# gooofy/zerovox

Measured on AMD Instinct MI355X. Metric: audio samples/sec + RTF, 128-phoneme zero-shot synth @22.05kHz, 1/2/4/8 GPU, higher is better.
Workload: dtype f16+bf16

## Files before the change

zerovox_amd/csrc/gemm.hip:

```cpp
#include "mfma_util.h"
#include "zvx_kernels.h"

#include <cstring>
#include <type_traits>

#ifndef ZVX_GEMM_PART
#define ZVX_GEMM_PART 0
#endif
#define ZVX_PART_MAIN (ZVX_GEMM_PART != 2)
#define ZVX_PART_RESFUSE (ZVX_GEMM_PART != 1)
#if ZVX_GEMM_PART == 2
extern thread_local bool zvx_gemm_dry_run;
#else
thread_local hipEvent_t zvx_gemm_ev_start = nullptr, zvx_gemm_ev_stop = nullptr;
thread_local bool zvx_gemm_dry_run = false;
#endif
#define g_dry_run zvx_gemm_dry_run

#define ZVX_LAUNCH(...) do { if (!g_dry_run) ZVX_DISPATCH(__VA_ARGS__); } while (0)

namespace zvx {


#define PITCH 80
// ... 1792 lines not shown
        dim3 grid((a.N / 128) * ((a.M + 255) / 256), a.nbatch);
        size_t lds = ((size_t)(256 + hl + hr) * SLAB_PITCH + 1023) & ~(size_t)1023;
        ZVX_LAUNCH((convslab_kernel<256, 128, 2, 2, true, 2, 0, -1, 160>), grid, dim3(256), lds, stream, a);
        return 7;
    }
    if (a.dtype != DT_F32 && a.N == a.K && !a.K2 && (a.ntaps == 3 || a.ntaps == 5 || a.ntaps == 7 || a.ntaps == 11)) {
        if (a.N == 32 && launch_convreg_c<32, 512, 4, 1, 2>(a, stream)) return 14;
        if (a.N == 64 && launch_convreg_c<64, 256, 2, 2, 2>(a, stream)) return 15;
    }
    if (hl + hr > 64) {
        if (hl + hr <= 160 && a.N % 128 == 0 && a.K % SLAB_KC == 0 && !a.K2 && !a.bflat && !a.flat_win && gemm_epi_mode_of(a) == ZVX_EPI(1, 1, 1)) {
            dim3 grid((a.N / 128) * ((a.M + 255) / 256), a.nbatch);
            const size_t lds = ((size_t)(256 + hl + hr) * SLAB_PITCH + 1023) & ~(size_t)1023;
            if (a.dtype == DT_F16) ZVX_LAUNCH((convslab_kernel<256, 128, 2, 2, true, 2, 0, ZVX_EPI(1, 1, 1), 160, true>), grid, dim3(256), lds, stream, a);
            else ZVX_LAUNCH((convslab_kernel<256, 128, 2, 2, true, 2, 0, ZVX_EPI(1, 1, 1), 160>), grid, dim3(256), lds, stream, a);
            return 7;
        }
        return -4;
    }
    static const int bns[4] = {256, 128, 64, 32};
    static const double eff[4] = {0.95, 1.0, 0.7, 0.4};
    int best = 0; double best_cost = -1;
    for (int i = 0; i < 4; i++) {
        const double cost = (double)((a.N + bns[i] - 1) / bns[i]) * bns[i] / eff[i];
        if (best_cost < 0 || cost < best_cost - 1e-9) { best_cost = cost; best = i; }
    }
    static const int bms[4] = {128, 256, 256, 256};
    const int ncu = num_cus();
    if (g_slab_small >= 2 && a.M <= 64 && a.nbatch * ((a.N + 127) / 128) * 4 <= ncu && a.N >= 64 && hl + hr <= 64) {
        a.bflat = 0;
        dim3 g32((a.N + 31) / 32, a.nbatch);
        const size_t lds32 = (((size_t)(256 + hl + hr) * SLAB_PITCH + 1023) & ~(size_t)1023) + (size_t)8 * 1024;
        launch_slab_variant<256, 32, 4, 1, 2, 8>(a, g32, lds32, stream);
        return 9;
    }
    if (g_slab_small && a.M > 128 && a.N >= 128 && hl + hr <= 64) {
        const long wg256 = (long)((a.N + 127) / 128) * ((a.M + 255) / 256) * a.nbatch;
        if (wg256 * 2 <= ncu) {
            a.bflat = 0;
            const bool r64 = wg256 * 4 <= ncu;
            const int bm = r64 ? 64 : 128;
            dim3 gs(((a.N + 127) / 128) * ((a.M + bm - 1) / bm), a.nbatch);
            size_t lds = ((size_t)(bm + hl + hr) * SLAB_PITCH + 1023) & ~(size_t)1023;
            const size_t stage = (size_t)4 * 32 * (2 * 128 + 16);
            if (lds < stage) lds = stage;
            if (r64) launch_slab_variant<64, 128, 2, 2, 2, 0>(a, gs, lds, stream);
            else launch_slab_variant<128, 128, 2, 2, 2, 0>(a, gs, lds, stream);
            return 22;
        }
    }
    if (a.M <= 128 && a.N >= 128) {
        a.bflat = 0;
        const int wide = ((a.N + 255) / 256) * a.nbatch;
        const bool narrow = wide < 2 * ncu;
        const int bn = narrow ? 128 : 256;
        dim3 grid((a.N + bn - 1) / bn, a.nbatch);
        size_t lds = ((size_t)(128 + hl + hr) * SLAB_PITCH + 1023) & ~(size_t)1023;
        const size_t stage = (size_t)4 * 32 * (2 * 128 + 16);
        if (lds < stage) lds = stage;
        if (narrow && a.M > (g_slab_small ? 32 : 64) && ((a.N + 127) / 128) * a.nbatch < 2 * ncu) {
            dim3 g64(((a.N + 127) / 128) * ((a.M + 63) / 64), a.nbatch);
            launch_slab_variant<64, 128, 2, 2, 2, 0>(a, g64, lds, stream);
            return 22;
        }
        if (narrow) { launch_slab_variant<128, 128, 2, 2, 2, 0>(a, grid, lds, stream); return 22; }
        launch_slab_variant<128, 256, 1, 4, 2, 0>(a, grid, lds, stream);
        return 6;
    }
    if (a.ntaps == 1 && a.N >= 512) {
        const long slots = 2L * ncu;
        auto rounds = [&](int bm_, int bn_) {
            const long ntn_ = (a.N + bn_ - 1) / bn_, utt = ntn_ * ((a.M + bm_ - 1) / bm_) * a.nbatch;
            const long flat = a.bflat ? ntn_ * (((long)a.nbatch * a.bflat + bm_ - 1) / bm_) : utt;
            return ((flat < utt ? flat : utt) + slots - 1) / slots;
        };
        best = rounds(256, 128) <= rounds(128, 256) ? 1 : 0;
    }
    const bool wreg = best <= 1;
    const int ring_slots = wreg ? 0 : (best == 0 ? 4 : 8);
    const int bn = bns[best], bm = bms[best];
    const int ntn = (a.N + bn - 1) / bn;
    if (a.bflat) {
        const long slots = 2L * ncu;
        const long wg_utt = (long)ntn * ((a.M + bm - 1) / bm) * a.nbatch, wg_flat = (long)ntn * (((long)a.nbatch * a.bflat + bm - 1) / bm);
        if ((wg_flat + slots - 1) / slots < (wg_utt + slots - 1) / slots) { a.flat_win = a.bflat; a.flat_rows = a.nbatch * a.bflat; a.M = a.flat_rows; a.nbatch = 1; }
        else a.bflat = 0;
    }
    if (best == 1 && bflat_hint && a.M > 256 && hl + hr <= 64) {
        const long slots = 2L * ncu;
        const long t256 = (long)ntn * ((a.M + 255) / 256) * a.nbatch, t128 = (long)ntn * ((a.M + 127) / 128) * a.nbatch;
        const long eff256 = 2 * ((t256 + slots - 1) / slots), eff128 = (t128 + slots - 1) / slots;
        if (eff128 < eff256) {
            dim3 g128(ntn * ((a.M + 127) / 128), a.nbatch);
            size_t lds128 = ((size_t)(128 + hl + hr) * SLAB_PITCH + 1023) & ~(size_t)1023;
            const size_t stage128 = (size_t)4 * 32 * (2 * 128 + 16);
            if (lds128 < stage128) lds128 = stage128;
            switch (gemm_epi_mode_of(a)) {
                case ZVX_EPI(0, 0, 1): launch_slab_variant<128, 128, 2, 2, 2, 0, ZVX_EPI(0, 0, 1)>(a, g128, lds128, stream); break;
                case ZVX_EPI_DEC(0): launch_slab_variant<128, 128, 2, 2, 2, 0, ZVX_EPI_DEC(0)>(a, g128, lds128, stream); break;
                case ZVX_EPI_DEC(1): launch_slab_variant<128, 128, 2, 2, 2, 0, ZVX_EPI_DEC(1)>(a, g128, lds128, stream); break;
                default: launch_slab_variant<128, 128, 2, 2, 2, 0>(a, g128, lds128, stream);
            }
            return 22;
        }
    }
    const int ntm = (a.M + bm - 1) / bm;
    dim3 grid(ntn * ntm, a.nbatch);
// ... 105 lines not shown
```

zerovox_amd/csrc/pairstream.hip:

```cpp
#include "mfma_util.h"
#include "zvx_kernels.h"

#include <algorithm>
#include <type_traits>

namespace zvx {

#define PS_R 128
#define PS_WD 8
#define PS_XP 256
#define PS_TP 272
#define PS_NDMA 8

#ifndef PS_EXP
#define PS_EXP 0
#endif
#ifndef PS_PD
#define PS_PD 2
#endif
#ifndef PS_PRIO
#define PS_PRIO 1
#endif
#ifndef PS_RES_LDS
#define PS_RES_LDS 1
#endif
#ifndef PS_RPF
#define PS_RPF 2
#endif
#ifndef PS_DMA_TAIL
#define PS_DMA_TAIL 1
#endif
#ifdef PS_PROFILE
#define PS_STAMP(k) do { const unsigned long long t_ = __builtin_readcyclecounter(); tacc[k] += t_ - tlast; tlast = t_; } while (0)
#else
#define PS_STAMP(k) do {} while (0)
#endif

template <int ROLE, int NT, int AM, bool HAS_OUT, bool H16>
__device__ __forceinline__ void ps_role(const PairArgs& a, unsigned char* lds, const int lane, const int ct) {
    constexpr int R = PS_R, H2 = (NT - 1) / 2, NS = 8 * NT, WD = PS_WD;
    constexpr int EPI = (ROLE == 0 && !PS_DMA_TAIL) ? (PS_NDMA + NT - 2) / (NT - 1) : 0;
    static_assert(ROLE == 1 || PS_DMA_TAIL || EPI * (NT - 1) >= PS_NDMA, "DMA slots");
    const int l32 = lane & 31, hi = lane >> 5;
    const int dil = a.dil, H1 = dil * H2, DX = a.DX, DT = a.DT, G0 = a.G0;
    const unsigned tbase = (unsigned)DX * PS_XP;
    const float* const bias_l = (const float*)(lds + tbase + (unsigned)DT * PS_TP) + ROLE * 128;
    const unsigned scratch_l = tbase + (unsigned)DT * PS_TP + 1024;

    const unsigned char* const wq = (const unsigned char*)(ROLE ? a.W2 : a.W1) + (long)ct * NS * 1024;
    const unsigned lane16 = lane * 16;
    u32x4 wreg[WD] = {};
    auto wload = [&](int off, int slot) __attribute__((always_inline)) {
        asm volatile("global_load_dwordx4 %0, %1, %2" : "+v"(wreg[slot]) : "v"(lane16), "s"(wq + off) : "memory");
    };
#pragma unroll
    for (int i = 0; i < WD; i++) wload(i * 1024, i);

    const float slope1 = a.slope1, rinv = a.res_inv_slope, oscale = a.out_scale, oslope = a.slope;
    f32x16 acc[4];
#ifdef PS_PROFILE
    unsigned long long tacc[4] = {0, 0, 0, 0}, tlast = __builtin_readcyclecounter();
#endif

    const int nsegs = a.nseg * a.nbatch;
    for (int seg = blockIdx.x; seg < nsegs; seg += gridDim.x) {
        const int b = seg / a.nseg, sj = seg - b * a.nseg;
        int len = a.len ? a.len[b] : a.M;
        len = __builtin_amdgcn_readfirstlane(len);
        const int seg0 = sj * a.S;
        if (seg0 >= len) continue;
        const int seg_end = min(seg0 + a.S, len);
        const int nb = (seg_end - seg0 + 2 * H2 + R - 1) / R;
        const int c1_0 = seg0 - H2;
        const int xrow0 = c1_0 - H1;
        const unsigned short* const Xb = (const unsigned short*)a.X + (long)b * a.x_bs;

        auto dma_rsrc = [&](int grow, bool real) __attribute__((always_inline)) {
            const unsigned long long pa = (unsigned long long)(Xb + (long)grow * a.ldx);
            int nrec = real ? (len - grow) * a.ldx * 2 : 0; if (nrec < 0) nrec = 0;
            return (i32x4){__builtin_amdgcn_readfirstlane((int)(unsigned)pa), __builtin_amdgcn_readfirstlane((int)((pa >> 32) & 0xffff)),
                           __builtin_amdgcn_readfirstlane(nrec), 0x00020000};
        };
        auto dma_piece = [&](const i32x4& rsrc, int grow, int pos, int pc, bool real) __attribute__((always_inline)) {
            int lv = lane;
            asm volatile("" : "+v"(lv));
            const int rr = lv >> 4, sl = lv & 15;
            int p = pos + 4 * pc; if (p >= DX) p -= DX;
            const int key = (p + rr) & 15;
            int voff = ((4 * pc + rr) * a.ldx + ((sl ^ key) << 3)) * 2;
            if (grow + 4 * pc + rr < 0) voff = -16;
            const unsigned la = __builtin_amdgcn_readfirstlane(real ? (unsigned)p * PS_XP : scratch_l);
            asm volatile("s_mov_b32 m0, %0\n\ts_nop 0\n\tbuffer_load_dwordx4 %1, %2, 0 offen lds" :: "s"(la), "v"(voff), "s"(rsrc) : "memory", "m0");
        };

        int x_rd = 0;
        int x_wr = G0;
        int gx = xrow0 + G0;
        int t_wr = 0;
        int t_rd = DT - 2 * H2;
        int g1 = c1_0;
        int g2 = seg0 - 2 * H2;
        if (ROLE == 0) {
            const i32x4 rs0 = dma_rsrc(xrow0, true);
            for (int pc = ct; pc < G0 / 4; pc += 4) dma_piece(rs0, xrow0, 0, pc, true);
            asm volatile("s_waitcnt vmcnt(0)" ::: "memory");
        }
        asm volatile("s_waitcnt lgkmcnt(0)\n\ts_barrier" ::: "memory");

        auto main_loop = [&](bool dma_real) __attribute__((always_inline)) {
#pragma unroll
            for (int j = 0; j < 4; j++)
#pragma unroll
                for (int e = 0; e < 16; e++) acc[j][e] = 0.f;
            unsigned bs[4], nbs[4], pn = 0, hkn = 0;
            auto bases_common = [&](int u) __attribute__((always_inline)) {
                const int kc = u >= NT ? 1 : 0, tap = u - kc * NT;
                if (ROLE == 0) {
                    pn = x_rd + l32 + tap * dil; pn = min(pn, pn - (unsigned)DX);
                    hkn = (((pn ^ hi) & 15u) << 4) ^ ((unsigned)kc << 7);
                } else {
                    pn = t_rd + l32 + tap; pn = min(pn, pn - (unsigned)DT);
                    hkn = tbase + hi * 16 + kc * 128;
                }
            };
            auto bases_tile = [&](int j, unsigned (&o)[4]) __attribute__((always_inline)) {
                unsigned pj = pn + 32 * j;
                if (ROLE == 0) { pj = min(pj, pj - (unsigned)DX); o[j] = (pj << 8) + hkn; }
                else { pj = min(pj, pj - (unsigned)DT); o[j] = pj * PS_TP + hkn; }
            };
            auto rd1 = [&](uint4& xf, unsigned o, int kk) __attribute__((always_inline)) {
                if (PS_EXP & 2) { asm volatile("" : "=v"(xf)); return; }
                if (PS_EXP & 64) {
                    uint4 dummy;
                    if (ROLE == 0) asm volatile("ds_read_b128 %0, %1" : "=v"(dummy) : "v"(o ^ (unsigned)(kk << 5)));
                    else asm volatile("ds_read_b128 %0, %1" : "=v"(dummy) : "v"(o + kk * 32));
                    asm volatile("" : "=v"(xf));
                    return;
                }
                if (ROLE == 0) asm volatile("ds_read_b128 %0, %1" : "=v"(xf) : "v"(o ^ (unsigned)(kk << 5)));
                else {
                    switch (kk) {
                        case 0: asm volatile("ds_read_b128 %0, %1" : "=v"(xf) : "v"(o)); break;
                        case 1: asm volatile("ds_read_b128 %0, %1 offset:32" : "=v"(xf) : "v"(o)); break;
                        case 2: asm volatile("ds_read_b128 %0, %1 offset:64" : "=v"(xf) : "v"(o)); break;
                        default: asm volatile("ds_read_b128 %0, %1 offset:96" : "=v"(xf) : "v"(o)); break;
                    }
                }
            };
            constexpr int PD = PS_PD;
            static_assert(PD == 1 || PD == 2, "prefetch distance");
            uint4 xs[4][4];
            const i32x4 rsd = PS_DMA_TAIL ? (i32x4){0, 0, 0, 0} : dma_rsrc(gx, dma_real);
            bases_common(0);
#pragma unroll
            for (int j = 0; j < 4; j++) bases_tile(j, bs);
            asm volatile("s_waitcnt lgkmcnt(0)" ::: "memory");
            __builtin_amdgcn_sched_barrier(0);
#pragma unroll
            for (int i = 0; i < PD; i++)
#pragma unroll
                for (int j = 0; j < 4; j++) rd1(xs[i][j], bs[j], i);
            for (int u2 = 0; u2 < NT; u2++) {
                const int next_off = (u2 + 1 == NT ? 0 : (u2 + 1) * (WD * 1024));
#pragma unroll
                for (int h = 0; h < 2; h++) {
                    const int u = 2 * u2 + h;
                    int un = u + 1; if (un == 2 * NT) un = 0;
#pragma unroll
                    for (int kk = 0; kk < 4; kk++) {
                        const int i = h * 4 + kk;
                        asm volatile("s_waitcnt vmcnt(%0) lgkmcnt(%1)" :: "n"(WD - 1 + EPI), "n"(4 * (PD - 1)) : "memory");
                        __builtin_amdgcn_sched_barrier(0);
#pragma unroll
                        for (int j = 0; j < 4; j++) {
                            if (PS_EXP & 32) asm volatile("" : "+v"(acc[j]) : "v"(wreg[i]), "v"(xs[i & 3][j]));
                            else acc[j] = mfma16<H16>(wreg[i], xs[i & 3][j], acc[j]);
                            __builtin_amdgcn_sched_barrier(0);
                            if (kk + PD < 4) rd1(xs[(i + PD) & 3][j], bs[j], kk + PD); else rd1(xs[(i + PD) & 3][j], nbs[j], kk + PD - 4);
                            if (kk == 0 && j == 3) bases_common(un);
                            if (kk == 1) bases_tile(j, nbs);
                            if (j == 3) {
                                if (!(PS_EXP & 1)) wload(next_off + i * 1024, i);
                                if (ROLE == 0 && !PS_DMA_TAIL && !(PS_EXP & 8)) {
#pragma unroll
                                    for (int e = 0; e < EPI; e++)
                                        if (i == (7 * e + 3) / EPI) {
                                            const int pidx = u2 * EPI + e;
                                            dma_piece(rsd, gx, x_wr, ct * PS_NDMA + (pidx < PS_NDMA ? pidx : 0), dma_real && pidx < PS_NDMA);
                                        }
                                }
                            }
                            __builtin_amdgcn_sched_barrier(0);
                        }
                    }
#pragma unroll
                    for (int j = 0; j < 4; j++) bs[j] = nbs[j];
                }
            }
            asm volatile("s_waitcnt lgkmcnt(0)" ::: "memory");
            __builtin_amdgcn_sched_barrier(0);
        };

        auto epilogue_T = [&]() __attribute__((always_inline)) {
            int lv = lane;
            asm volatile("" : "+v"(lv));
            const int l32 = lv & 31, hi = lv >> 5;
            float4 bq[4];
#pragma unroll
            for (int q = 0; q < 4; q++) bq[q] = *(const float4*)(bias_l + ct * 32 + 8 * q + 4 * hi);
#pragma unroll
            for (int j = 0; j < 4; j++) {
                const int g = g1 + 32 * j + l32;
                const bool inside = g >= 0 && g < len;
                unsigned wp = t_wr + 32 * j + l32; wp = min(wp, wp - (unsigned)DT);
                unsigned char* const dst = lds + tbase + wp * PS_TP + (ct * 32 + 4 * hi) * 2;
#pragma unroll
                for (int q = 0; q < 4; q++) {
                    const f32x2 v01 = lrelu2((f32x2){acc[j][4 * q], acc[j][4 * q + 1]} + (f32x2){bq[q].x, bq[q].y}, slope1);
                    const f32x2 v23 = lrelu2((f32x2){acc[j][4 * q + 2], acc[j][4 * q + 3]} + (f32x2){bq[q].z, bq[q].w}, slope1);
                    uint2 pk;
                    pk.x = inside ? pack16<H16>(v01.x, v01.y) : 0u;
                    pk.y = inside ? pack16<H16>(v23.x, v23.y) : 0u;
                    if (!(PS_EXP & 16)) *(uint2*)(dst + q * 16) = pk;
                    else asm volatile("" :: "v"(pk.x), "v"(pk.y), "v"(dst));
                }
            }
        };

        int off[4];
        u32x4 rx[4][2], sx[4][2];
        uint2 rcur[4][4], rnext[4][4];
        auto residual_reads = [&](int blk) __attribute__((always_inline)) {
            int lv = lane;
            asm volatile("" : "+v"(lv));
            unsigned p0 = (unsigned)((long)blk * R % DX) + H1 - H2 + (lv & 31);
            p0 = min(p0, p0 - (unsigned)DX);
#pragma unroll
            for (int j = 0; j < 4; j++) {
                unsigned pj = p0 + 32 * j; pj = min(pj, pj - (unsigned)DX);
                const unsigned char* row = lds + pj * PS_XP + (lv >> 5) * 8;
#pragma unroll
                for (int q = 0; q < 4; q++) rnext[j][q] = *(const uint2*)(row + (((ct * 4 + q) ^ (pj & 15u)) << 4));
            }
        };
        auto res_rsrc = [&](const void* base, long bs_) __attribute__((always_inline)) {
            return __builtin_amdgcn_make_buffer_rsrc((void*)((unsigned short*)base + (long)b * bs_), 0, len * a.ldx * 2, 0x00020000);
        };
        auto epilogue_loads = [&](int gb) __attribute__((always_inline)) {
            int lv = lane;
            asm volatile("" : "+v"(lv));
            const int cA = ct * 32 + 8 * (lv >> 5);
            const __amdgpu_buffer_rsrc_t rsX = res_rsrc(a.X, a.x_bs), rsA = res_rsrc(a.accum, a.a_bs);
#pragma unroll
            for (int j = 0; j < 4; j++) {
                const int g = gb + 32 * j + (lv & 31);
                off[j] = (g >= seg0 && g < seg_end && !(PS_EXP & 4)) ? (g * a.ldx + cA) * 2 : (int)0x80000000;
                if (!PS_RES_LDS) {
                    rx[j][0] = __builtin_amdgcn_raw_buffer_load_b128(rsX, off[j], 0, 0);
                    rx[j][1] = __builtin_amdgcn_raw_buffer_load_b128(rsX, off[j] + 32, 0, 0);
                }
            }
            if (AM & 1) {
#pragma unroll
                for (int j = 0; j < 4; j++) {
                    sx[j][0] = __builtin_amdgcn_raw_buffer_load_b128(rsA, off[j], 0, 0);
                    sx[j][1] = __builtin_amdgcn_raw_buffer_load_b128(rsA, off[j] + 32, 0, 0);
                }
            }
        };
        auto epilogue_out = [&]() __attribute__((always_inline)) {
            int lv = lane;
            asm volatile("" : "+v"(lv));
            float4 bq[4];
#pragma unroll
            for (int q = 0; q < 4; q++) bq[q] = *(const float4*)(bias_l + ct * 32 + 8 * q + 4 * (lv >> 5));
            const __amdgpu_buffer_rsrc_t rsA = res_rsrc(a.accum, a.a_bs), rsO = res_rsrc(a.out, a.o_bs);
#pragma unroll
            for (int j = 0; j < 4; j++) {
                float v[16];
#pragma unroll
                for (int q = 0; q < 4; q++) {
                    v[4 * q] = acc[j][4 * q] + bq[q].x; v[4 * q + 1] = acc[j][4 * q + 1] + bq[q].y;
                    v[4 * q + 2] = acc[j][4 * q + 2] + bq[q].z; v[4 * q + 3] = acc[j][4 * q + 3] + bq[q].w;
                    if (PS_RES_LDS) {
                        const f32x2 r01 = inv_lrelu2(unpack16<H16>(rcur[j][q].x), rinv), r23 = inv_lrelu2(unpack16<H16>(rcur[j][q].y), rinv);
                        v[4 * q] += r01.x; v[4 * q + 1] += r01.y; v[4 * q + 2] += r23.x; v[4 * q + 3] += r23.y;
                    }
                }
#pragma unroll
                for (int pr = 0; pr < 2; pr++) {
                    float w8[8];
#pragma unroll
                    for (int e = 0; e < 4; e++) {
                        const auto r = __builtin_amdgcn_permlane32_swap(__float_as_uint(v[8 * pr + e]), __float_as_uint(v[8 * pr + 4 + e]), false, false);
                        w8[e] = __uint_as_float(r[0]); w8[4 + e] = __uint_as_float(r[1]);
                    }
                    f32x2 t[4] = {(f32x2){w8[0], w8[1]}, (f32x2){w8[2], w8[3]}, (f32x2){w8[4], w8[5]}, (f32x2){w8[6], w8[7]}};
                    if (!PS_RES_LDS) {
                        const u32x4 rr = rx[j][pr];
                        t[0] += inv_lrelu2(unpack16<H16>(rr.x), rinv); t[1] += inv_lrelu2(unpack16<H16>(rr.y), rinv);
                        t[2] += inv_lrelu2(unpack16<H16>(rr.z), rinv); t[3] += inv_lrelu2(unpack16<H16>(rr.w), rinv);
                    }
                    if (AM & 1) {
                        const u32x4 ss = sx[j][pr];
                        t[0] += unpack16<H16>(ss.x); t[1] += unpack16<H16>(ss.y); t[2] += unpack16<H16>(ss.z); t[3] += unpack16<H16>(ss.w);
                    }
                    if (AM & 2)
                        __builtin_amdgcn_raw_buffer_store_b128((u32x4){pack16<H16>(t[0].x, t[0].y), pack16<H16>(t[1].x, t[1].y), pack16<H16>(t[2].x, t[2].y), pack16<H16>(t[3].x, t[3].y)},
                                                               rsA, off[j] + 32 * pr, 0, 0);
                    if (HAS_OUT) {
                        if (AM) {
#pragma unroll
                            for (int e = 0; e < 4; e++) t[e] *= oscale;
                        }
#pragma unroll
                        for (int e = 0; e < 4; e++) t[e] = lrelu2(t[e], oslope);
                        __builtin_amdgcn_raw_buffer_store_b128((u32x4){pack16<H16>(t[0].x, t[0].y), pack16<H16>(t[1].x, t[1].y), pack16<H16>(t[2].x, t[2].y), pack16<H16>(t[3].x, t[3].y)},
                                                               rsO, off[j] + 32 * pr, 0, 0);
                    }
                }
            }
        };

        for (int s = 0; s <= nb + 1; s++) {
            if (ROLE == 0) {
                if (s < nb) {
                    main_loop(s + 1 < nb);
                    if (PS_DMA_TAIL && !(PS_EXP & 8) && s + 1 < nb) {
                        const i32x4 rsd = dma_rsrc(gx, true);
#pragma unroll
                        for (int pc = 0; pc < PS_NDMA; pc++) dma_piece(rsd, gx, x_wr, ct * PS_NDMA + pc, true);
                    }
                    PS_STAMP(0);
                    gx += R; x_wr += R; if (x_wr >= DX) x_wr -= DX;
                    if (PS_PRIO & 2) __builtin_amdgcn_s_setprio(2);
                    epilogue_T();
                    if (PS_PRIO & 2) __builtin_amdgcn_s_setprio(0);
                    PS_STAMP(1);
                    x_rd += R; if (x_rd >= DX) x_rd -= DX;
                    t_wr += R; if (t_wr >= DT) t_wr -= DT;
                    g1 += R;
                }
            } else {
                if (s >= 2) {
                    if (PS_PRIO & 1) __builtin_amdgcn_s_setprio(2);
                    if (!PS_RPF) epilogue_loads(g2);
                    epilogue_out();
                    if (PS_PRIO & 1) __builtin_amdgcn_s_setprio(0);
                    g2 += R;
                    PS_STAMP(1);
                }
                if (PS_RES_LDS) {
#pragma unroll
                    for (int j = 0; j < 4; j++)
#pragma unroll
                        for (int q = 0; q < 4; q++) rcur[j][q] = rnext[j][q];
                    residual_reads(s);
                }
                if (s >= 1 && s <= nb) {
                    if (PS_RPF == 1) epilogue_loads(g2);
                    main_loop(false);
                    if (PS_RPF == 2) epilogue_loads(g2);
                    t_rd += R; if (t_rd >= DT) t_rd -= DT;
                    PS_STAMP(0);
                }
            }
            if (PS_DMA_TAIL && ROLE == 0 && s < nb) asm volatile("s_waitcnt vmcnt(0)" ::: "memory");
            if (s <= nb) asm volatile("s_waitcnt lgkmcnt(0)\n\ts_barrier" ::: "memory");
            PS_STAMP(2);
        }
    }
#pragma unroll
    for (int i = 0; i < WD; i++) asm volatile("s_waitcnt vmcnt(0)" : "+v"(wreg[i]) :: "memory");
#ifdef PS_PROFILE
    if (a.prof && blockIdx.x == 0 && lane == 0)
        for (int k = 0; k < 4; k++) a.prof[(ROLE * 4 + ct) * 4 + k] = (long long)tacc[k];
#endif
}

template <int NT, int AM, bool HAS_OUT, bool H16>
__global__ __launch_bounds__(512) __attribute__((amdgpu_waves_per_eu(2, 2))) void pairstream128_kernel(const PairArgs a) {
    if (H16) f16_saturate_mode();
    extern __shared__ __attribute__((aligned(256))) unsigned char lds[];
    const int tid = threadIdx.x, lane = tid & 63, wave = __builtin_amdgcn_readfirstlane(tid >> 6);
    float* const bias_l = (float*)(lds + (unsigned)a.DX * PS_XP + (unsigned)a.DT * PS_TP);
    if (tid < 256) bias_l[tid] = tid < 128 ? a.b1[tid] : a.b2[tid - 128];
    __syncthreads();
    asm volatile("s_waitcnt vmcnt(0)" ::: "memory");
    if (wave < 4) ps_role<0, NT, AM, HAS_OUT, H16>(a, lds, lane, wave);
    else ps_role<1, NT, AM, HAS_OUT, H16>(a, lds, lane, wave - 4);
}

static int ps_ncu() { return persistent_cus(); }

bool launch_pairstream(PairArgs a, hipStream_t stream, bool dry_run) {
    if (a.C != 128 || a.ldx != a.C || a.dil < 1 || !a.W1 || !a.W2 || !a.b1 || !a.b2) return false;
    if (!(a.ntaps == 3 || a.ntaps == 7 || a.ntaps == 11)) return false;
    if ((a.out && a.ldo != a.ldx) || (a.accum && a.lda != a.ldx)) return false;
    if ((long)a.M * a.ldx * 2 >= (1l << 31)) return false;
    const int am = a.accum ? a.accum_mode : 0;
    if (!a.out && !(am & 2)) return false;
    if (a.out && am >= 2) return false;
    const int H2 = (a.ntaps - 1) / 2, H1 = a.dil * H2;
    a.G0 = (PS_R + 2 * H1 + 3) & ~3;
    a.DX = (a.G0 + PS_R + 15) & ~15;
    a.DT = 2 * PS_R + 2 * H2;
    const size_t lds = (size_t)a.DX * PS_XP + (size_t)a.DT * PS_TP + 1024 + 1024;
    if (lds > 160 * 1024 || 4 * PS_NDMA * 4 != PS_R) return false;
    const long rows_all = (long)a.M * a.nbatch;
    const int nwg = ps_ncu();
    if (rows_all < (long)nwg * 768 && !a.force) return false;
    int S = (int)((rows_all + nwg - 1) / nwg);
    if (S < 1024) S = 1024;
    S = (S + PS_R - 1) / PS_R * PS_R;
    a.S = S; a.nseg = (a.M + S - 1) / S;
    if (dry_run) return true;
    const int nsegs = a.nseg * a.nbatch;
    const dim3 grid(nsegs < nwg ? nsegs : nwg), block(512);
#define PS_GO1(NT_, AM_, HO_, H_) do { auto kfn = pairstream128_kernel<NT_, AM_, HO_, H_>; \
        if (!lds_opt_in((const void*)kfn)) return false; \
        ZVX_DISPATCH(kfn, grid, block, lds, stream, a); return true; } while (0)
#define PS_GO(NT_, AM_, HO_) do { if (a.f16) PS_GO1(NT_, AM_, HO_, true); else PS_GO1(NT_, AM_, HO_, false); } while (0)
#define PS_MODE(NT_) do { if (a.out) { if (am == 0) PS_GO(NT_, 0, true); if (am == 1) PS_GO(NT_, 1, true); return false; } \
        if (am == 2) PS_GO(NT_, 2, false); if (am == 3) PS_GO(NT_, 3, false); return false; } while (0)
    if (a.ntaps == 3) PS_MODE(3);
    if (a.ntaps == 7) PS_MODE(7);
    if (a.ntaps == 11) PS_MODE(11);
#undef PS_MODE
#undef PS_GO
#undef PS_GO1
    return false;
}

}
```

zerovox_amd/csrc/zvx_kernels.h:

```cpp
#pragma once
#include <hip/hip_runtime.h>
#include <hip/hip_ext.h>
#include <stdint.h>
#include <atomic>
#include <mutex>
#include <set>
#include <utility>

extern thread_local hipEvent_t zvx_gemm_ev_start, zvx_gemm_ev_stop;
#define ZVX_DISPATCH(kernel, grid, block, lds, stream, ...) \
    do { if (zvx_gemm_ev_start) hipExtLaunchKernelGGL(kernel, grid, block, lds, stream, zvx_gemm_ev_start, zvx_gemm_ev_stop, 0, __VA_ARGS__); \
         else hipLaunchKernelGGL(kernel, grid, block, lds, stream, __VA_ARGS__); } while (0)

namespace zvx {

inline void profile_events(hipEvent_t start, hipEvent_t stop) { zvx_gemm_ev_start = start; zvx_gemm_ev_stop = stop; }

typedef unsigned short bf16_t;

enum DType { DT_F32 = 0, DT_BF16 = 1, DT_F16 = 2 };
static inline size_t dtype_size(int dt) { return dt == DT_F32 ? 4 : 2; }
inline int num_cus() {
    static const int n = [] { int dev = 0, v = 0; if (hipGetDevice(&dev) != hipSuccess || hipDeviceGetAttribute(&v, hipDeviceAttributeMultiprocessorCount, dev) != hipSuccess || v <= 0) v = 256; return v; }();
    return n;
// ... 44 lines not shown
    float res_inv_slope;
    void* accum; long a_bs; int lda; int accum_mode;
    int accum_dtype;
    float out_scale;
    int act; float slope;
    const float* post_scale; const float* post_shift;
    void* out; long o_bs, o_hs; int ldo; int out_dtype;
    float* se_part; int* se_part_S;
    void* ds_out; const void* ds_Wp; const float* ds_bias;
    double flops;
};

int launch_gemm(const GemmArgs& a, hipStream_t stream);
int gemm_variant_of(const GemmArgs& a);
int gemm_epi_mode_of(const GemmArgs& a);
int launch_resfuse(GemmArgs a, hipStream_t stream);
int launch_rb2fuse(GemmArgs a, hipStream_t stream);
size_t packed_weight_elems(int ntaps, int N, int K);
void launch_pack_pair(const void* packedA, int ntapsA, int KA, const void* packedB, int ntapsB, int KB, int N, void* out, hipStream_t s);
void launch_pack_weights(const void* w_bf16, int ntaps, int N, int K, void* out, hipStream_t s);
const char* gemm_variant_name(int id);
int gemm_num_variants();

struct StreamArgs {
    const void* X; long x_bs; int ldx;
    const void* W1[3]; const void* W2[3];
    const float* b1[3]; const float* b2[3];
    int dil[3];
    int C, ntaps, npair;
    void* out; long o_bs; int ldo;
    void* accum; long a_bs; int lda; int accum_mode;
    float slope1, res_inv_slope, out_scale, slope;
    const int* len; int M, nbatch;
    int S, nseg;
    int dX0, dT, dX[3];
    double flops;
    long long* prof;
    int seg_min;
    int f16;
};
int launch_resstream(StreamArgs a, hipStream_t stream, bool dry_run);

struct PairArgs {
    const void* X; long x_bs; int ldx;
    const void* W1; const void* W2;
    const float* b1; const float* b2;
    int C, ntaps, dil;
    void* out; long o_bs; int ldo;
    void* accum; long a_bs; int lda; int accum_mode;
    float slope1, res_inv_slope, out_scale, slope;
    const int* len; int M, nbatch;
    int force;
    int f16;
    int S, nseg, DX, DT, G0;
    long long* prof;
};
bool launch_pairstream(PairArgs a, hipStream_t stream, bool dry_run);

struct StageArgs {
    const void* X; long x_bs; int ldx;
    const void* W;
    int woff[18];
    const float* bias;
    int C, nk, ks[3], dil[3][3];
    void* out; long o_bs; int ldo;
    float slope1, res_inv_slope, slope;
    const int* len; int M, nbatch;
    int f16;
};
bool launch_narrowstage(const StageArgs& a, hipStream_t stream, bool dry_run);
int narrowstage_steps(int C, int k);
void launch_pack_narrow(const void* w16 , int k, int C, void* out, hipStream_t s);

struct FlashArgs {
    const void* qk; long qk_bs; int ldq; int k_off;
    const void* vt; long vt_bs; int ldv;
    void* out; long o_bs; int ldo;
    const int* len; int L, D, nheads, nbatch;
    float scale;
    int f16;
    long long* prof;
};
bool launch_flash_attention(const FlashArgs& a, hipStream_t stream, bool dry_run);
struct AttnF32Args {
    const float* qkv; long bs; int ld; int q_off, k_off, v_off;
    float* out; long o_bs; int ldo;
    unsigned short* planes; int planes_C;
    int planes_f16;
    const int* len; int L, D, nheads, nbatch;
    float scale;
};
bool launch_attention_f32(const AttnF32Args& a, hipStream_t stream, bool dry_run);

struct LoudCoef { double b0, b1, b2, a1, a2, c1, c2; };
constexpr int LEVEL_TILE = 4096;
constexpr int LEVEL_MAX_S = 600;
constexpr int LEVEL_MIN_H = 400;
constexpr int LEVEL_NODES = LEVEL_TILE / LEVEL_MIN_H + 4;
struct LevelRow {
    const float* x; void* out; double* p;
    long in_origin;
    long q_first, q_last;
    long U;
    int n, off, cnt, pad_;
};
constexpr long LEVEL_OPEN = 0x7fffffffffffffffL;
// ... 233 lines not shown
```

Baseline: 347.5 million.

## Add optional wide pairstream variant with two channel tiles per wave

Templates the pairstream role on NCT so that each wave can compute two 32-channel tiles, reusing each X fragment across two weight tiles. A 256-thread wide kernel using this is added behind PS_WIDE, which defaults to 0, and a runtime flag. Separately, the slab GEMM dispatch now forces the narrow 128-column tile whenever it accumulates into an f16 buffer. The wide path doubles register pressure and drops priority tweaks. The gemm narrow-tile change is active by default.

Result: no change. 347.5 million, median of 2 (-0.0%).

```diff
diff --git a/zerovox_amd/csrc/gemm.hip b/zerovox_amd/csrc/gemm.hip
--- a/zerovox_amd/csrc/gemm.hip
+++ b/zerovox_amd/csrc/gemm.hip
@@ -1868,7 +1868,7 @@
     if (a.M <= 128 && a.N >= 128) {
         a.bflat = 0;
         const int wide = ((a.N + 255) / 256) * a.nbatch;
-        const bool narrow = wide < 2 * ncu;
+        const bool narrow = wide < 2 * ncu || (a.accum_mode && a.accum && a.accum_dtype == DT_F16);
         const int bn = narrow ? 128 : 256;
         dim3 grid((a.N + bn - 1) / bn, a.nbatch);
         size_t lds = ((size_t)(128 + hl + hr) * SLAB_PITCH + 1023) & ~(size_t)1023;
diff --git a/zerovox_amd/csrc/pairstream.hip b/zerovox_amd/csrc/pairstream.hip
--- a/zerovox_amd/csrc/pairstream.hip
+++ b/zerovox_amd/csrc/pairstream.hip
@@ -27,6 +27,9 @@
 #ifndef PS_RPF
 #define PS_RPF 2
 #endif
+#ifndef PS_WIDE
+#define PS_WIDE 0
+#endif
 #ifndef PS_DMA_TAIL
 #define PS_DMA_TAIL 1
 #endif
@@ -36,9 +39,13 @@
 #define PS_STAMP(k) do {} while (0)
 #endif
 
-template <int ROLE, int NT, int AM, bool HAS_OUT, bool H16>
-__device__ __forceinline__ void ps_role(const PairArgs& a, unsigned char* lds, const int lane, const int ct) {
+template <int ROLE, int NT, int AM, bool HAS_OUT, bool H16, int NCT>
+__device__ __forceinline__ void ps_role(const PairArgs& a, unsigned char* lds, const int lane, const int cw) {
     constexpr int R = PS_R, H2 = (NT - 1) / 2, NS = 8 * NT, WD = PS_WD;
+    constexpr int NW = 4 / NCT, NDMA = PS_NDMA * NCT;
+    constexpr int PRIO = NCT == 1 ? PS_PRIO : 0;
+    static_assert(NCT == 1 || (NCT == 2 && PS_DMA_TAIL), "channel tiles per wave");
+    const int ct0 = cw * NCT;
     constexpr int EPI = (ROLE == 0 && !PS_DMA_TAIL) ? (PS_NDMA + NT - 2) / (NT - 1) : 0;
     static_assert(ROLE == 1 || PS_DMA_TAIL || EPI * (NT - 1) >= PS_NDMA, "DMA slots");
     const int l32 = lane & 31, hi = lane >> 5;
@@ -47,17 +54,19 @@
     const float* const bias_l = (const float*)(lds + tbase + (unsigned)DT * PS_TP) + ROLE * 128;
     const unsigned scratch_l = tbase + (unsigned)DT * PS_TP + 1024;
 
-    const unsigned char* const wq = (const unsigned char*)(ROLE ? a.W2 : a.W1) + (long)ct * NS * 1024;
+    const unsigned char* const wq = (const unsigned char*)(ROLE ? a.W2 : a.W1) + (long)ct0 * NS * 1024;
     const unsigned lane16 = lane * 16;
-    u32x4 wreg[WD] = {};
+    u32x4 wreg[WD * NCT] = {};
     auto wload = [&](int off, int slot) __attribute__((always_inline)) {
         asm volatile("global_load_dwordx4 %0, %1, %2" : "+v"(wreg[slot]) : "v"(lane16), "s"(wq + off) : "memory");
     };
 #pragma unroll
-    for (int i = 0; i < WD; i++) wload(i * 1024, i);
+    for (int i = 0; i < WD; i++)
+#pragma unroll
+        for (int c = 0; c < NCT; c++) wload(c * (NS * 1024) + i * 1024, i * NCT + c);
 
     const float slope1 = a.slope1, rinv = a.res_inv_slope, oscale = a.out_scale, oslope = a.slope;
-    f32x16 acc[4];
+    f32x16 acc[NCT][4];
 #ifdef PS_PROFILE
     unsigned long long tacc[4] = {0, 0, 0, 0}, tlast = __builtin_readcyclecounter();
 #endif
@@ -102,16 +111,18 @@
         int g2 = seg0 - 2 * H2;
         if (ROLE == 0) {
             const i32x4 rs0 = dma_rsrc(xrow0, true);
-            for (int pc = ct; pc < G0 / 4; pc += 4) dma_piece(rs0, xrow0, 0, pc, true);
+            for (int pc = cw; pc < G0 / 4; pc += NW) dma_piece(rs0, xrow0, 0, pc, true);
             asm volatile("s_waitcnt vmcnt(0)" ::: "memory");
         }
         asm volatile("s_waitcnt lgkmcnt(0)\n\ts_barrier" ::: "memory");
 
         auto main_loop = [&](bool dma_real) __attribute__((always_inline)) {
 #pragma unroll
-            for (int j = 0; j < 4; j++)
-#pragma unroll
-                for (int e = 0; e < 16; e++) acc[j][e] = 0.f;
+            for (int c = 0; c < NCT; c++)
+#pragma unroll
+                for (int j = 0; j < 4; j++)
+#pragma unroll
+                    for (int e = 0; e < 16; e++) acc[c][j][e] = 0.f;
             unsigned bs[4], nbs[4], pn = 0, hkn = 0;
             auto bases_common = [&](int u) __attribute__((always_inline)) {
                 const int kc = u >= NT ? 1 : 0, tap = u - kc * NT;
@@ -169,24 +180,30 @@
 #pragma unroll
                     for (int kk = 0; kk < 4; kk++) {
                         const int i = h * 4 + kk;
-                        asm volatile("s_waitcnt vmcnt(%0) lgkmcnt(%1)" :: "n"(WD - 1 + EPI), "n"(4 * (PD - 1)) : "memory");
+                        asm volatile("s_waitcnt vmcnt(%0) lgkmcnt(%1)" :: "n"(NCT * (WD - 1) + EPI), "n"(4 * (PD - 1)) : "memory");
                         __builtin_amdgcn_sched_barrier(0);
 #pragma unroll
                         for (int j = 0; j < 4; j++) {
-                            if (PS_EXP & 32) asm volatile("" : "+v"(acc[j]) : "v"(wreg[i]), "v"(xs[i & 3][j]));
-                            else acc[j] = mfma16<H16>(wreg[i], xs[i & 3][j], acc[j]);
+#pragma unroll
+                            for (int c = 0; c < NCT; c++) {
+                                if (PS_EXP & 32) asm volatile("" : "+v"(acc[c][j]) : "v"(wreg[i * NCT + c]), "v"(xs[i & 3][j]));
+                                else acc[c][j] = mfma16<H16>(wreg[i * NCT + c], xs[i & 3][j], acc[c][j]);
+                            }
                             __builtin_amdgcn_sched_barrier(0);
                             if (kk + PD < 4) rd1(xs[(i + PD) & 3][j], bs[j], kk + PD); else rd1(xs[(i + PD) & 3][j], nbs[j], kk + PD - 4);
                             if (kk == 0 && j == 3) bases_common(un);
                             if (kk == 1) bases_tile(j, nbs);
                             if (j == 3) {
-                                if (!(PS_EXP & 1)) wload(next_off + i * 1024, i);
+                                if (!(PS_EXP & 1)) {
+#pragma unroll
+                                    for (int c = 0; c < NCT; c++) wload(c * (NS * 1024) + next_off + i * 1024, i * NCT + c);
+                                }
                                 if (ROLE == 0 && !PS_DMA_TAIL && !(PS_EXP & 8)) {
 #pragma unroll
                                     for (int e = 0; e < EPI; e++)
                                         if (i == (7 * e + 3) / EPI) {
                                             const int pidx = u2 * EPI + e;
-                                            dma_piece(rsd, gx, x_wr, ct * PS_NDMA + (pidx < PS_NDMA ? pidx : 0), dma_real && pidx < PS_NDMA);
+                                            dma_piece(rsd, gx, x_wr, cw * PS_NDMA + (pidx < PS_NDMA ? pidx : 0), dma_real && pidx < PS_NDMA);
                                         }
                                 }
                             }
@@ -205,31 +222,34 @@
             int lv = lane;
             asm volatile("" : "+v"(lv));
             const int l32 = lv & 31, hi = lv >> 5;
-            float4 bq[4];
-#pragma unroll
-            for (int q = 0; q < 4; q++) bq[q] = *(const float4*)(bias_l + ct * 32 + 8 * q + 4 * hi);
-#pragma unroll
-            for (int j = 0; j < 4; j++) {
-                const int g = g1 + 32 * j + l32;
-                const bool inside = g >= 0 && g < len;
-                unsigned wp = t_wr + 32 * j + l32; wp = min(wp, wp - (unsigned)DT);
-                unsigned char* const dst = lds + tbase + wp * PS_TP + (ct * 32 + 4 * hi) * 2;
-#pragma unroll
-                for (int q = 0; q < 4; q++) {
-                    const f32x2 v01 = lrelu2((f32x2){acc[j][4 * q], acc[j][4 * q + 1]} + (f32x2){bq[q].x, bq[q].y}, slope1);
-                    const f32x2 v23 = lrelu2((f32x2){acc[j][4 * q + 2], acc[j][4 * q + 3]} + (f32x2){bq[q].z, bq[q].w}, slope1);
-                    uint2 pk;
-                    pk.x = inside ? pack16<H16>(v01.x, v01.y) : 0u;
-                    pk.y = inside ? pack16<H16>(v23.x, v23.y) : 0u;
-                    if (!(PS_EXP & 16)) *(uint2*)(dst + q * 16) = pk;
-                    else asm volatile("" :: "v"(pk.x), "v"(pk.y), "v"(dst));
+#pragma unroll
+            for (int c = 0; c < NCT; c++) {
+                float4 bq[4];
+#pragma unroll
+                for (int q = 0; q < 4; q++) bq[q] = *(const float4*)(bias_l + (ct0 + c) * 32 + 8 * q + 4 * hi);
+#pragma unroll
+                for (int j = 0; j < 4; j++) {
+                    const int g = g1 + 32 * j + l32;
+                    const bool inside = g >= 0 && g < len;
+                    unsigned wp = t_wr + 32 * j + l32; wp = min(wp, wp - (unsigned)DT);
+                    unsigned char* const dst = lds + tbase + wp * PS_TP + ((ct0 + c) * 32 + 4 * hi) * 2;
+#pragma unroll
+                    for (int q = 0; q < 4; q++) {
+                        const f32x2 v01 = lrelu2((f32x2){acc[c][j][4 * q], acc[c][j][4 * q + 1]} + (f32x2){bq[q].x, bq[q].y}, slope1);
+                        const f32x2 v23 = lrelu2((f32x2){acc[c][j][4 * q + 2], acc[c][j][4 * q + 3]} + (f32x2){bq[q].z, bq[q].w}, slope1);
+                        uint2 pk;
+                        pk.x = inside ? pack16<H16>(v01.x, v01.y) : 0u;
+                        pk.y = inside ? pack16<H16>(v23.x, v23.y) : 0u;
+                        if (!(PS_EXP & 16)) *(uint2*)(dst + q * 16) = pk;
+                        else asm volatile("" :: "v"(pk.x), "v"(pk.y), "v"(dst));
+                    }
                 }
             }
         };
 
         int off[4];
-        u32x4 rx[4][2], sx[4][2];
-        uint2 rcur[4][4], rnext[4][4];
+        u32x4 rx[NCT][4][2], sx[NCT][4][2];
+        uint2 rcur[NCT][4][4], rnext[NCT][4][4];
         auto residual_reads = [&](int blk) __attribute__((always_inline)) {
             int lv = lane;
             asm volatile("" : "+v"(lv));
@@ -240,7 +260,9 @@
                 unsigned pj = p0 + 32 * j; pj = min(pj, pj - (unsigned)DX);
                 const unsigned char* row = lds + pj * PS_XP + (lv >> 5) * 8;
 #pragma unroll
-                for (int q = 0; q < 4; q++) rnext[j][q] = *(const uint2*)(row + (((ct * 4 + q) ^ (pj & 15u)) << 4));
+                for (int c = 0; c < NCT; c++)
+#pragma unroll
+                    for (int q = 0; q < 4; q++) rnext[c][j][q] = *(const uint2*)(row + ((((ct0 + c) * 4 + q) ^ (pj & 15u)) << 4));
             }
         };
         auto res_rsrc = [&](const void* base, long bs_) __attribute__((always_inline)) {
@@ -249,74 +271,82 @@
         auto epilogue_loads = [&](int gb) __attribute__((always_inline)) {
             int lv = lane;
             asm volatile("" : "+v"(lv));
-            const int cA = ct * 32 + 8 * (lv >> 5);
+            const int cA = ct0 * 32 + 8 * (lv >> 5);
             const __amdgpu_buffer_rsrc_t rsX = res_rsrc(a.X, a.x_bs), rsA = res_rsrc(a.accum, a.a_bs);
 #pragma unroll
             for (int j = 0; j < 4; j++) {
                 const int g = gb + 32 * j + (lv & 31);
                 off[j] = (g >= seg0 && g < seg_end && !(PS_EXP & 4)) ? (g * a.ldx + cA) * 2 : (int)0x80000000;
                 if (!PS_RES_LDS) {
-                    rx[j][0] = __builtin_amdgcn_raw_buffer_load_b128(rsX, off[j], 0, 0);
-                    rx[j][1] = __builtin_amdgcn_raw_buffer_load_b128(rsX, off[j] + 32, 0, 0);
+#pragma unroll
+                    for (int c = 0; c < NCT; c++) {
+                        rx[c][j][0] = __builtin_amdgcn_raw_buffer_load_b128(rsX, off[j] + 64 * c, 0, 0);
+                        rx[c][j][1] = __builtin_amdgcn_raw_buffer_load_b128(rsX, off[j] + 64 * c + 32, 0, 0);
+                    }
                 }
             }
             if (AM & 1) {
 #pragma unroll
-                for (int j = 0; j < 4; j++) {
-                    sx[j][0] = __builtin_amdgcn_raw_buffer_load_b128(rsA, off[j], 0, 0);
-                    sx[j][1] = __builtin_amdgcn_raw_buffer_load_b128(rsA, off[j] + 32, 0, 0);
-                }
+                for (int c = 0; c < NCT; c++)
+#pragma unroll
+                    for (int j = 0; j < 4; j++) {
+                        sx[c][j][0] = __builtin_amdgcn_raw_buffer_load_b128(rsA, off[j] + 64 * c, 0, 0);
+                        sx[c][j][1] = __builtin_amdgcn_raw_buffer_load_b128(rsA, off[j] + 64 * c + 32, 0, 0);
+                    }
             }
         };
         auto epilogue_out = [&]() __attribute__((always_inline)) {
             int lv = lane;
             asm volatile("" : "+v"(lv));
-            float4 bq[4];
-#pragma unroll
-            for (int q = 0; q < 4; q++) bq[q] = *(const float4*)(bias_l + ct * 32 + 8 * q + 4 * (lv >> 5));
             const __amdgpu_buffer_rsrc_t rsA = res_rsrc(a.accum, a.a_bs), rsO = res_rsrc(a.out, a.o_bs);
 #pragma unroll
-            for (int j = 0; j < 4; j++) {
-                float v[16];
-#pragma unroll
-                for (int q = 0; q < 4; q++) {
-                    v[4 * q] = acc[j][4 * q] + bq[q].x; v[4 * q + 1] = acc[j][4 * q + 1] + bq[q].y;
-                    v[4 * q + 2] = acc[j][4 * q + 2] + bq[q].z; v[4 * q + 3] = acc[j][4 * q + 3] + bq[q].w;
-                    if (PS_RES_LDS) {
-                        const f32x2 r01 = inv_lrelu2(unpack16<H16>(rcur[j][q].x), rinv), r23 = inv_lrelu2(unpack16<H16>(rcur[j][q].y), rinv);
-                        v[4 * q] += r01.x; v[4 * q + 1] += r01.y; v[4 * q + 2] += r23.x; v[4 * q + 3] += r23.y;
-                    }
-                }
-#pragma unroll
-                for (int pr = 0; pr < 2; pr++) {
-                    float w8[8];
-#pragma unroll
-                    for (int e = 0; e < 4; e++) {
-                        const auto r = __builtin_amdgcn_permlane32_swap(__float_as_uint(v[8 * pr + e]), __float_as_uint(v[8 * pr + 4 + e]), false, false);
-                        w8[e] = __uint_as_float(r[0]); w8[4 + e] = __uint_as_float(r[1]);
-                    }
-                    f32x2 t[4] = {(f32x2){w8[0], w8[1]}, (f32x2){w8[2], w8[3]}, (f32x2){w8[4], w8[5]}, (f32x2){w8[6], w8[7]}};
-                    if (!PS_RES_LDS) {
-                        const u32x4 rr = rx[j][pr];
-                        t[0] += inv_lrelu2(unpack16<H16>(rr.x), rinv); t[1] += inv_lrelu2(unpack16<H16>(rr.y), rinv);
-                        t[2] += inv_lrelu2(unpack16<H16>(rr.z), rinv); t[3] += inv_lrelu2(unpack16<H16>(rr.w), rinv);
-                    }
-                    if (AM & 1) {
-                        const u32x4 ss = sx[j][pr];
-                        t[0] += unpack16<H16>(ss.x); t[1] += unpack16<H16>(ss.y); t[2] += unpack16<H16>(ss.z); t[3] += unpack16<H16>(ss.w);
-                    }
-                    if (AM & 2)
-                        __builtin_amdgcn_raw_buffer_store_b128((u32x4){pack16<H16>(t[0].x, t[0].y), pack16<H16>(t[1].x, t[1].y), pack16<H16>(t[2].x, t[2].y), pack16<H16>(t[3].x, t[3].y)},
-                                                               rsA, off[j] + 32 * pr, 0, 0);
-                    if (HAS_OUT) {
-                        if (AM) {
-#pragma unroll
-                            for (int e = 0; e < 4; e++) t[e] *= oscale;
+            for (int c = 0; c < NCT; c++) {
+                float4 bq[4];
+#pragma unroll
+                for (int q = 0; q < 4; q++) bq[q] = *(const float4*)(bias_l + (ct0 + c) * 32 + 8 * q + 4 * (lv >> 5));
+#pragma unroll
+                for (int j = 0; j < 4; j++) {
+                    float v[16];
+#pragma unroll
+                    for (int q = 0; q < 4; q++) {
+                        v[4 * q] = acc[c][j][4 * q] + bq[q].x; v[4 * q + 1] = acc[c][j][4 * q + 1] + bq[q].y;
+                        v[4 * q + 2] = acc[c][j][4 * q + 2] + bq[q].z; v[4 * q + 3] = acc[c][j][4 * q + 3] + bq[q].w;
+                        if (PS_RES_LDS) {
+                            const f32x2 r01 = inv_lrelu2(unpack16<H16>(rcur[c][j][q].x), rinv), r23 = inv_lrelu2(unpack16<H16>(rcur[c][j][q].y), rinv);
+                            v[4 * q] += r01.x; v[4 * q + 1] += r01.y; v[4 * q + 2] += r23.x; v[4 * q + 3] += r23.y;
                         }
-#pragma unroll
-                        for (int e = 0; e < 4; e++) t[e] = lrelu2(t[e], oslope);
-                        __builtin_amdgcn_raw_buffer_store_b128((u32x4){pack16<H16>(t[0].x, t[0].y), pack16<H16>(t[1].x, t[1].y), pack16<H16>(t[2].x, t[2].y), pack16<H16>(t[3].x, t[3].y)},
-                                                               rsO, off[j] + 32 * pr, 0, 0);
+                    }
+#pragma unroll
+                    for (int pr = 0; pr < 2; pr++) {
+                        float w8[8];
+#pragma unroll
+                        for (int e = 0; e < 4; e++) {
+                            const auto r = __builtin_amdgcn_permlane32_swap(__float_as_uint(v[8 * pr + e]), __float_as_uint(v[8 * pr + 4 + e]), false, false);
+                            w8[e] = __uint_as_float(r[0]); w8[4 + e] = __uint_as_float(r[1]);
+                        }
+                        f32x2 t[4] = {(f32x2){w8[0], w8[1]}, (f32x2){w8[2], w8[3]}, (f32x2){w8[4], w8[5]}, (f32x2){w8[6], w8[7]}};
+                        if (!PS_RES_LDS) {
+                            const u32x4 rr = rx[c][j][pr];
+                            t[0] += inv_lrelu2(unpack16<H16>(rr.x), rinv); t[1] += inv_lrelu2(unpack16<H16>(rr.y), rinv);
+                            t[2] += inv_lrelu2(unpack16<H16>(rr.z), rinv); t[3] += inv_lrelu2(unpack16<H16>(rr.w), rinv);
+                        }
+                        if (AM & 1) {
+                            const u32x4 ss = sx[c][j][pr];
+                            t[0] += unpack16<H16>(ss.x); t[1] += unpack16<H16>(ss.y); t[2] += unpack16<H16>(ss.z); t[3] += unpack16<H16>(ss.w);
+                        }
+                        if (AM & 2)
+                            __builtin_amdgcn_raw_buffer_store_b128((u32x4){pack16<H16>(t[0].x, t[0].y), pack16<H16>(t[1].x, t[1].y), pack16<H16>(t[2].x, t[2].y), pack16<H16>(t[3].x, t[3].y)},
+                                                                   rsA, off[j] + 64 * c + 32 * pr, 0, 0);
+                        if (HAS_OUT) {
+                            if (AM) {
+#pragma unroll
+                                for (int e = 0; e < 4; e++) t[e] *= oscale;
+                            }
+#pragma unroll
+                            for (int e = 0; e < 4; e++) t[e] = lrelu2(t[e], oslope);
+                            __builtin_amdgcn_raw_buffer_store_b128((u32x4){pack16<H16>(t[0].x, t[0].y), pack16<H16>(t[1].x, t[1].y), pack16<H16>(t[2].x, t[2].y), pack16<H16>(t[3].x, t[3].y)},
+                                                                   rsO, off[j] + 64 * c + 32 * pr, 0, 0);
+                        }
                     }
                 }
             }
@@ -329,32 +359,53 @@
                     if (PS_DMA_TAIL && !(PS_EXP & 8) && s + 1 < nb) {
                         const i32x4 rsd = dma_rsrc(gx, true);
 #pragma unroll
-                        for (int pc = 0; pc < PS_NDMA; pc++) dma_piece(rsd, gx, x_wr, ct * PS_NDMA + pc, true);
+                        for (int pc = 0; pc < NDMA; pc++) dma_piece(rsd, gx, x_wr, cw * NDMA + pc, true);
                     }
                     PS_STAMP(0);
                     gx += R; x_wr += R; if (x_wr >= DX) x_wr -= DX;
-                    if (PS_PRIO & 2) __builtin_amdgcn_s_setprio(2);
+                    if (PRIO & 2) __builtin_amdgcn_s_setprio(2);
                     epilogue_T();
-                    if (PS_PRIO & 2) __builtin_amdgcn_s_setprio(0);
+                    if (PRIO & 2) __builtin_amdgcn_s_setprio(0);
                     PS_STAMP(1);
                     x_rd += R; if (x_rd >= DX) x_rd -= DX;
                     t_wr += R; if (t_wr >= DT) t_wr -= DT;
                     g1 += R;
                 }
+            } else if (NCT == 2) {
+                if (s >= 1 && s <= nb) {
+                    main_loop(false);
+                    t_rd += R; if (t_rd >= DT) t_rd -= DT;
+                    PS_STAMP(0);
+                    epilogue_loads(g2);
+                    epilogue_out();
+                    g2 += R;
+                    PS_STAMP(1);
+                }
+                if (PS_RES_LDS && s < nb) {
+                    residual_reads(s);
+#pragma unroll
+                    for (int c = 0; c < NCT; c++)
+#pragma unroll
+                        for (int j = 0; j < 4; j++)
+#pragma unroll
+                            for (int q = 0; q < 4; q++) rcur[c][j][q] = rnext[c][j][q];
+                }
             } else {
                 if (s >= 2) {
-                    if (PS_PRIO & 1) __builtin_amdgcn_s_setprio(2);
+                    if (PRIO & 1) __builtin_amdgcn_s_setprio(2);
                     if (!PS_RPF) epilogue_loads(g2);
                     epilogue_out();
-                    if (PS_PRIO & 1) __builtin_amdgcn_s_setprio(0);
+                    if (PRIO & 1) __builtin_amdgcn_s_setprio(0);
                     g2 += R;
                     PS_STAMP(1);
                 }
                 if (PS_RES_LDS) {
 #pragma unroll
-                    for (int j = 0; j < 4; j++)
-#pragma unroll
-                        for (int q = 0; q < 4; q++) rcur[j][q] = rnext[j][q];
+                    for (int c = 0; c < NCT; c++)
+#pragma unroll
+                        for (int j = 0; j < 4; j++)
+#pragma unroll
+                            for (int q = 0; q < 4; q++) rcur[c][j][q] = rnext[c][j][q];
                     residual_reads(s);
                 }
                 if (s >= 1 && s <= nb) {
@@ -371,15 +422,16 @@
         }
     }
 #pragma unroll
-    for (int i = 0; i < WD; i++) asm volatile("s_waitcnt vmcnt(0)" : "+v"(wreg[i]) :: "memory");
+    for (int i = 0; i < WD * NCT; i++) asm volatile("s_waitcnt vmcnt(0)" : "+v"(wreg[i]) :: "memory");
 #ifdef PS_PROFILE
     if (a.prof && blockIdx.x == 0 && lane == 0)
-        for (int k = 0; k < 4; k++) a.prof[(ROLE * 4 + ct) * 4 + k] = (long long)tacc[k];
+        for (int k = 0; k < 4; k++) a.prof[(ROLE * 4 + ct0) * 4 + k] = (long long)tacc[k];
 #endif
 }
 
-template <int NT, int AM, bool HAS_OUT, bool H16>
-__global__ __launch_bounds__(512) __attribute__((amdgpu_waves_per_eu(2, 2))) void pairstream128_kernel(const PairArgs a) {
+template <int NT, int AM, bool HAS_OUT, bool H16, int NCT>
+__device__ __forceinline__ void ps_workgroup(const PairArgs& a) {
+    constexpr int NW = 4 / NCT;
     if (H16) f16_saturate_mode();
     extern __shared__ __attribute__((aligned(256))) unsigned char lds[];
     const int tid = threadIdx.x, lane = tid & 63, wave = __builtin_amdgcn_readfirstlane(tid >> 6);
@@ -387,9 +439,20 @@
     if (tid < 256) bias_l[tid] = tid < 128 ? a.b1[tid] : a.b2[tid - 128];
     __syncthreads();
     asm volatile("s_waitcnt vmcnt(0)" ::: "memory");
-    if (wave < 4) ps_role<0, NT, AM, HAS_OUT, H16>(a, lds, lane, wave);
-    else ps_role<1, NT, AM, HAS_OUT, H16>(a, lds, lane, wave - 4);
+    if (wave < NW) ps_role<0, NT, AM, HAS_OUT, H16, NCT>(a, lds, lane, wave);
+    else ps_role<1, NT, AM, HAS_OUT, H16, NCT>(a, lds, lane, wave - NW);
 }
+
+template <int NT, int AM, bool HAS_OUT, bool H16>
+__global__ __launch_bounds__(512) __attribute__((amdgpu_waves_per_eu(2, 2))) void pairstream128_kernel(const PairArgs a) {
+    ps_workgroup<NT, AM, HAS_OUT, H16, 1>(a);
+}
+#if PS_WIDE
+template <int NT, int AM, bool HAS_OUT, bool H16>
+__global__ __launch_bounds__(256) __attribute__((amdgpu_waves_per_eu(1, 1))) void pairstream128_wide_kernel(const PairArgs a) {
+    ps_workgroup<NT, AM, HAS_OUT, H16, 2>(a);
+}
+#endif
 
 static int ps_ncu() { return persistent_cus(); }
 
@@ -416,8 +479,15 @@
     a.S = S; a.nseg = (a.M + S - 1) / S;
     if (dry_run) return true;
     const int nsegs = a.nseg * a.nbatch;
-    const dim3 grid(nsegs < nwg ? nsegs : nwg), block(512);
-#define PS_GO1(NT_, AM_, HO_, H_) do { auto kfn = pairstream128_kernel<NT_, AM_, HO_, H_>; \
+#if PS_WIDE
+    const bool wide = a.wide != 0;
+#define PS_KFN(NT_, AM_, HO_, H_) (wide ? pairstream128_wide_kernel<NT_, AM_, HO_, H_> : pairstream128_kernel<NT_, AM_, HO_, H_>)
+#else
+    const bool wide = false;
+#define PS_KFN(NT_, AM_, HO_, H_) pairstream128_kernel<NT_, AM_, HO_, H_>
+#endif
+    const dim3 grid(nsegs < nwg ? nsegs : nwg), block(wide ? 256 : 512);
+#define PS_GO1(NT_, AM_, HO_, H_) do { auto kfn = PS_KFN(NT_, AM_, HO_, H_); \
         if (!lds_opt_in((const void*)kfn)) return false; \
         ZVX_DISPATCH(kfn, grid, block, lds, stream, a); return true; } while (0)
 #define PS_GO(NT_, AM_, HO_) do { if (a.f16) PS_GO1(NT_, AM_, HO_, true); else PS_GO1(NT_, AM_, HO_, false); } while (0)
@@ -429,6 +499,7 @@
 #undef PS_MODE
 #undef PS_GO
 #undef PS_GO1
+#undef PS_KFN
     return false;
 }
 
diff --git a/zerovox_amd/csrc/zvx_kernels.h b/zerovox_amd/csrc/zvx_kernels.h
--- a/zerovox_amd/csrc/zvx_kernels.h
+++ b/zerovox_amd/csrc/zvx_kernels.h
@@ -120,6 +120,7 @@
     const int* len; int M, nbatch;
     int force;
     int f16;
+    int wide;
     int S, nseg, DX, DT, G0;
     long long* prof;
 };
```
